# DHDev0/Stochastic-muzero

Hardware: AMD Instinct MI355X
Metric: MCTS simulations/sec (whole node), CartPole MLP 4096 envs × 50 sims (higher is better)
Workload: dtype f32 (tree values, heads) + f64 (pUCT scores, root priors) + i32 (counts)

## Files before the change

include/smz.h:

```cpp
#ifndef SMZ_H
#define SMZ_H

#include <stddef.h>
#include <stdint.h>

#ifdef __cplusplus
extern "C" {
#endif

#define SMZ_ABI_VERSION 1
#define SMZ_MAX_ACTIONS 32
#define SMZ_MAX_ACTIONS_LARGE 1024
#define SMZ_MAX_PLAYER_CYCLE 32
#define SMZ_MT_WORDS 624

typedef enum {
    SMZ_OK = 0,
    SMZ_ERR_INVALID = -1,
    SMZ_ERR_HIP = -2,
    SMZ_ERR_NOMEM = -3,
    SMZ_ERR_STATE = -4,
    SMZ_ERR_TOO_LARGE = -5
} smz_status;

// ... 65 lines not shown

int smz_expand_backup_select(smz_handle *h, const float *hidden_dev, const float *reward_dev, const float *policy_dev,
                             const float *value_dev, float *parent_hidden_dev, int32_t *last_action_dev,
                             uint8_t *branch_dev, float *mlp_input_dev, smz_stream stream);

int smz_root_stats(smz_handle *h, int32_t *visits_dev, double *priors_dev, float *root_value_dev,
                   float *child_reward_dev, smz_stream stream);

int smz_act(smz_handle *h, double temperature, const double *pow_table_host, int32_t *action_dev, double *policy_dev,
            double *child_visits_dev, float *root_value_dev, smz_stream stream);

int smz_support_decode(const float *logits_dev, int S, float *out_dev, int B, smz_stream stream);
int smz_policy_softmax(const float *logits_dev, int A, float *out_dev, int B, smz_stream stream);
int smz_dynamics_epilogue(const float *state_dyn_dev, const float *state_after_dev, const float *reward_logits_dev,
                          int ld, const uint8_t *branch_dev, int S, float *hidden_out_dev, float *reward_out_dev, int B,
                          smz_stream stream);
int smz_prediction_epilogue(const float *policy_logits_pred_dev, const float *value_logits_pred_dev,
                            const float *policy_logits_after_dev, const float *value_logits_after_dev, int ld,
                            const uint8_t *branch_dev, int A, int S, float *policy_out_dev, float *value_out_dev,
                            int B, smz_stream stream);

typedef struct {
    int32_t obs, A, S, H, L;
    int32_t OP;
    int32_t total_floats;
    int32_t off[30];
} smz_mlp_desc;
int smz_mlp_layout(smz_mlp_desc *desc);
int smz_mlp_initial(const smz_mlp_desc *desc, const float *weights_dev, const float *obs_dev, float *hidden_out_dev,
                    float *policy_out_dev, int B, smz_stream stream);
int smz_mlp_recurrent(const smz_mlp_desc *desc, const float *weights_dev, const float *mlp_input_dev,
                      const uint8_t *branch_dev, float *hidden_out_dev, float *reward_out_dev, float *policy_out_dev,
                      float *value_out_dev, int B, smz_stream stream);

enum { SMZ_LSTM_TRUNKS = 7, SMZ_LSTM_MAX_LAYERS = 4, SMZ_LSTM_REP = 2 * SMZ_LSTM_TRUNKS * SMZ_LSTM_MAX_LAYERS,
       SMZ_LSTM_OFFSETS = SMZ_LSTM_REP + 2, SMZ_LSTM_SLACK = 256 };
typedef struct {
    int32_t obs, A, S, L;
    int32_t total_floats;
    int32_t recurrent_floats;
    int32_t lds_bytes;
    int32_t off[SMZ_LSTM_OFFSETS];
} smz_lstm_desc;
int smz_lstm_layout(smz_lstm_desc *desc);
int smz_lstm_initial(const smz_lstm_desc *desc, const float *weights_dev, const float *obs_dev, float *hidden_out_dev,
                     float *policy_out_dev, int B, smz_stream stream);
int smz_lstm_recurrent(const smz_lstm_desc *desc, const float *weights_dev, const float *mlp_input_dev,
                       const uint8_t *branch_dev, float *hidden_out_dev, float *reward_out_dev, float *policy_out_dev,
                       float *value_out_dev, int B, smz_stream stream);

enum { SMZ_V_DYN = 0, SMZ_V_ADY = 1, SMZ_V_PRE = 2, SMZ_V_APR = 3 };
enum { SMZ_VT_CONV_IN = 0, SMZ_VT_BN_IN, SMZ_VT_RES_A, SMZ_VT_RES_B, SMZ_VT_RES_BN, SMZ_VT_MIX_W, SMZ_VT_MIX_B,
       SMZ_VT_TOWER , SMZ_V_TRANS_STRIDE = 13 };
enum { SMZ_VP_RES_A = 0, SMZ_VP_RES_B, SMZ_VP_RES_BN, SMZ_VP_VMIX_W, SMZ_VP_VMIX_B, SMZ_VP_VTOWER ,
       SMZ_VP_PMIX_W = 11, SMZ_VP_PMIX_B, SMZ_VP_PTOWER , SMZ_V_PRED_STRIDE = 19 };
enum { SMZ_VR_STEM = 0, SMZ_VR_NARROW_A, SMZ_VR_NARROW_B, SMZ_VR_NARROW_BN, SMZ_VR_WIDEN, SMZ_VR_WIDE_A, SMZ_VR_WIDE_B,
       SMZ_VR_WIDE_BN, SMZ_VR_LAST_A, SMZ_VR_LAST_B, SMZ_VR_LAST_BN };
enum { SMZ_V_TRANS_BASE = 0, SMZ_V_PRED_BASE = 26, SMZ_V_REP_BASE = 64, SMZ_V_OFFSETS = 80 };
typedef struct smz_vision_desc {
    int32_t A, S, H, L;
    int32_t OP;
    int32_t total_floats;
    int32_t small_floats;
    int32_t off[SMZ_V_OFFSETS];
} smz_vision_desc;
int smz_vision_layout(smz_vision_desc *desc);
// ... 141 lines not shown
```

stochastic-muzero_amd/_lib.py:

```python
import ctypes as C
import os

_HERE = os.path.dirname(os.path.abspath(__file__))
LIB_PATH = os.environ.get("SMZ_LIB_PATH") or os.path.join(_HERE, "libsmz.so")

SMZ_OK, SMZ_ERR_INVALID, SMZ_ERR_HIP, SMZ_ERR_NOMEM, SMZ_ERR_STATE, SMZ_ERR_TOO_LARGE = 0, -1, -2, -3, -4, -5
RNG_MT19937_NUMPY, RNG_PHILOX = 0, 1
MAX_ACTIONS = 32
MAX_ACTIONS_LARGE = 1024


class SmzError(RuntimeError):
    def __init__(self, code, text):
        super().__init__(f"libsmz error {code}: {text}")
        self.code = code


class Config(C.Structure):
    _fields_ = [("num_trees", C.c_int32), ("num_actions", C.c_int32), ("max_action_sample", C.c_int32),
                ("hidden_size", C.c_int32), ("num_simulations", C.c_int32), ("pb_c_base", C.c_int32),
                ("pb_c_init", C.c_double), ("discount", C.c_double), ("root_dirichlet_alpha", C.c_double),
                ("root_exploration_fraction", C.c_double), ("rng_mode", C.c_int32), ("device", C.c_int32)]


# ... 30 lines not shown


_P = C.c_void_p
SIGNATURES = {
    "smz_create": (C.c_int, [C.POINTER(Config), C.POINTER(_P)]),
    "smz_create_large_actions": (C.c_int, [C.POINTER(Config), C.POINTER(_P)]),
    "smz_destroy": (C.c_int, [_P]),
    "smz_abi_version": (C.c_int, []),
    "smz_build_features": (C.c_int, []),
    "smz_last_error": (C.c_char_p, []),
    "smz_node_capacity": (C.c_int, [_P]),
    "smz_last_kernel": (C.c_int, [_P, C.c_char_p, C.c_int]),
    "smz_set_pb_c_table": (C.c_int, [_P, _P, C.c_int]),
    "smz_seed": (C.c_int, [_P, _P, _P]),
    "smz_set_rng_state": (C.c_int, [_P, C.c_int, _P, C.c_int]),
    "smz_get_rng_state": (C.c_int, [_P, C.c_int, _P, C.POINTER(C.c_int)]),
    "smz_philox_words": (C.c_int, [C.c_uint64, C.c_uint32, C.c_int, C.c_int, _P]),
    "smz_get_philox_position": (C.c_int, [_P, C.c_int, C.POINTER(C.c_uint32), C.POINTER(C.c_int)]),
    "smz_rng_snapshot": (C.c_int, [_P, _P]),
    "smz_rng_restore": (C.c_int, [_P, _P]),
    "smz_root_init": (C.c_int, [_P, _P, _P, _P, C.c_int, _P]),
    "smz_select": (C.c_int, [_P, _P, _P, _P, _P, _P]),
    "smz_expand_backup": (C.c_int, [_P, _P, _P, _P, _P, _P]),
    "smz_expand_backup_select": (C.c_int, [_P, _P, _P, _P, _P, _P, _P, _P, _P, _P]),
    "smz_root_stats": (C.c_int, [_P, _P, _P, _P, _P, _P]),
    "smz_act": (C.c_int, [_P, C.c_double, _P, _P, _P, _P, _P, _P]),
    "smz_support_decode": (C.c_int, [_P, C.c_int, _P, C.c_int, _P]),
    "smz_policy_softmax": (C.c_int, [_P, C.c_int, _P, C.c_int, _P]),
    "smz_dynamics_epilogue": (C.c_int, [_P, _P, _P, C.c_int, _P, C.c_int, _P, _P, C.c_int, _P]),
    "smz_prediction_epilogue": (C.c_int, [_P, _P, _P, _P, C.c_int, _P, C.c_int, C.c_int, _P, _P, C.c_int, _P]),
    "smz_mlp_layout": (C.c_int, [C.POINTER(MlpDesc)]),
    "smz_mlp_initial": (C.c_int, [C.POINTER(MlpDesc), _P, _P, _P, _P, C.c_int, _P]),
    "smz_mlp_recurrent": (C.c_int, [C.POINTER(MlpDesc), _P, _P, _P, _P, _P, _P, _P, C.c_int, _P]),
    "smz_mlp_layout_wide": (C.c_int, [C.POINTER(MlpDesc)]),
    "smz_mlp_recurrent_wide": (C.c_int, [C.POINTER(MlpDesc), _P, _P, _P, _P, _P, _P, _P, C.c_int, _P]),
    "smz_mlp_layout_large": (C.c_int, [C.POINTER(MlpDesc)]),
    "smz_mlp_recurrent_large": (C.c_int, [C.POINTER(MlpDesc), _P, _P, _P, _P, _P, _P, _P, _P, C.c_int, _P]),
    "smz_mlp_initial_wide": (C.c_int, [C.POINTER(MlpDesc), _P, _P, _P, _P, C.c_int, _P]),
    "smz_mlp_initial_large": (C.c_int, [C.POINTER(MlpDesc), _P, _P, _P, _P, C.c_int, _P]),
    "smz_lstm_layout": (C.c_int, [C.POINTER(LstmDesc)]),
    "smz_lstm_initial": (C.c_int, [C.POINTER(LstmDesc), _P, _P, _P, _P, C.c_int, _P]),
    "smz_lstm_recurrent": (C.c_int, [C.POINTER(LstmDesc), _P, _P, _P, _P, _P, _P, _P, C.c_int, _P]),
    "smz_vision_layout": (C.c_int, [C.POINTER(VisionDesc)]),
    "smz_vision_initial": (C.c_int, [C.POINTER(VisionDesc), _P, _P, _P, _P, C.c_int, _P]),
    "smz_vision_initial_record": (C.c_int, [C.POINTER(VisionDesc), _P, _P, _P, _P, _P, C.c_int, _P]),
    "smz_vision_recurrent": (C.c_int, [C.POINTER(VisionDesc), _P, _P, C.c_int, _P, _P, _P, _P, _P, _P, C.c_int, _P]),
    "smz_search_mlp_act": (C.c_int, [_P, C.POINTER(MlpDesc), _P, _P, C.c_int, C.c_double, _P, _P, _P, _P, _P, _P]),
    "smz_search_mlp_act_cartpole": (C.c_int, [_P, C.POINTER(MlpDesc), _P, C.c_int, C.c_double, _P, _P, _P, _P, _P,
                                              C.POINTER(CartPoleEnv), _P]),
    "smz_search_mlp": (C.c_int, [_P, C.POINTER(MlpDesc), _P, _P, C.c_int, _P]),
    "smz_frames_resize_u8": (C.c_int, [_P, C.c_int, C.c_int, C.c_int, C.c_int, C.c_int, _P, _P, _P]),
    "smz_frames_resize_taps_u8": (C.c_int, [_P, C.c_int, C.c_int, C.c_int, C.c_int, C.c_int, _P, _P, _P]),
    "smz_host_register": (C.c_int, [_P, C.c_size_t]),
    "smz_host_unregister": (C.c_int, [_P]),
    "smz_copy_async": (C.c_int, [_P, _P, C.c_size_t, C.c_int, _P]),
    "smz_search_vision": (C.c_int, [_P, C.POINTER(VisionDesc), _P, _P, _P, C.c_int, _P]),
    "smz_search_vision_act": (C.c_int, [_P, C.POINTER(VisionDesc), _P, _P, _P, C.c_int, C.c_double, _P, _P, _P, _P, _P, _P]),
    "smz_search_lstm": (C.c_int, [_P, C.POINTER(LstmDesc), _P, _P, _P, C.c_int, _P]),
    "smz_search_lstm_act": (C.c_int, [_P, C.POINTER(LstmDesc), _P, _P, _P, C.c_int, C.c_double, _P, _P, _P, _P, _P, _P]),
    "smz_search_mlp_wide": (C.c_int, [_P, C.POINTER(MlpDesc), _P, _P, _P, C.c_int, _P]),
    "smz_search_mlp_wide_act": (C.c_int, [_P, C.POINTER(MlpDesc), _P, _P, _P, C.c_int, C.c_double, _P, _P, _P, _P, _P, _P]),
    "smz_search_mlp_large": (C.c_int, [_P, C.POINTER(MlpDesc), _P, _P, _P, C.c_int, _P]),
    "smz_search_mlp_large_act": (C.c_int, [_P, C.POINTER(MlpDesc), _P, _P, _P, C.c_int, C.c_double, _P, _P, _P, _P, _P, _P]),
    "smz_search_mlp_players": (C.c_int, [_P, C.POINTER(MlpDesc), _P, _P, C.c_int, _P]),
    "smz_search_mlp_players_act": (C.c_int, [_P, C.POINTER(MlpDesc), _P, _P, C.c_int, C.c_double, _P, _P, _P, _P, _P, _P]),
    "smz_cartpole_step": (C.c_int, [_P, _P, _P, _P, _P, C.c_int, _P]),
# ... 67 lines not shown
```

stochastic-muzero_amd/csrc/smz_mlp.hip:

```cpp
#include <hip/hip_runtime.h>
#include <math.h>
#include <stdint.h>
#include <stdlib.h>
#include <stdio.h>

#include "../../include/smz.h"
#include "smz_mlp_device.hpp"
#include "smz_mlp_wide_device.hpp"

using namespace smz_mlp;

namespace {

extern __shared__ float4 smz_mlp_lds4[];

constexpr int kFastS = 31, kFastH = 64, kFastL = 0;
template <int U, bool FASTD>
__global__ void __launch_bounds__(512) k_mlp_recurrent(smz_mlp_desc d, const float *weights, const float *x,
                                                       const uint8_t *branch, float *hidden_out, float *reward_out,
                                                       float *policy_out, float *value_out, int B, int rows_per_wave) {
    float *lds = reinterpret_cast<float *>(smz_mlp_lds4);
    stage_recurrent_weights(lds, weights, d);
    if (FASTD) { d.S = kFastS; d.H = kFastH; d.L = kFastL; d.OP = kWave; }
    const int lane = threadIdx.x & (kWave - 1), wave = threadIdx.x / kWave, waves = blockDim.x / kWave;
    float *scratch = lds + d.total_floats + wave * scratch_floats(d);
    const int row0 = (blockIdx.x * waves + wave) * rows_per_wave;
    const int S = d.S, A = d.A, K4in = up4(S + A), rs = row_scratch_floats(d);
    for (int i = 0; i < rows_per_wave; i += kRows) {
        if (row0 + i >= B) break;
        const float *xin[kRows];
        bool dyn[kRows], live[kRows];
        float *dh[kRows], *dp[kRows];
        float reward[kRows], value[kRows];
#pragma unroll
        for (int r = 0; r < kRows; r++) {
            const int row = row0 + i + r;
            live[r] = (i + r < rows_per_wave) && row < B;
            const int rr = live[r] ? row : row0 + i;
            float *xb = scratch + r * rs;
            for (int k = lane; k < K4in; k += kWave) xb[k] = (k < S + A) ? x[(size_t)rr * (S + A) + k] : 0.f;
            xin[r] = xb;
            dyn[r] = branch[rr] != 0;
            dh[r] = hidden_out + (size_t)rr * S;
            dp[r] = policy_out + (size_t)rr * A;
        }
        lds_sync();
        recurrent_rows<U, kRows>(lds, d, scratch, xin, dyn, live, dh, dp, reward, value);
#pragma unroll
        for (int r = 0; r < kRows; r++) {
            if (live[r] && lane == 0) {
                if (reward_out) reward_out[row0 + i + r] = reward[r];
                value_out[row0 + i + r] = value[r];
            }
        }
    }
}

template <int U>
__global__ void __launch_bounds__(512) k_mlp_initial(smz_mlp_desc d, const float *weights, const float *obs,
                                                     float *hidden_out, float *policy_out, int B, int rows_per_wave) {
    float *lds = reinterpret_cast<float *>(smz_mlp_lds4);
    stage_initial_weights(lds, weights, d);
    const int wave = threadIdx.x / kWave, waves = blockDim.x / kWave;
    float *scratch = lds + d.total_floats + wave * scratch_floats(d);
    const int row0 = (blockIdx.x * waves + wave) * rows_per_wave;
    for (int i = 0; i < rows_per_wave; i++) {
        const int row = row0 + i;
        if (row >= B) break;
        initial_row<U>(lds, d, lds, d, scratch, obs + (size_t)row * d.obs, hidden_out + (size_t)row * d.S, nullptr,
                       policy_out + (size_t)row * d.A);
    }
}

#ifndef SMZ_MFMA_COMPACT
#define SMZ_MFMA_COMPACT 1
#endif
constexpr bool kMfmaCompact = SMZ_MFMA_COMPACT != 0;
constexpr int kMfmaWaves = kMfmaCompact ? 16 : 12;
constexpr int kTileFloats = 32 * 32;

__device__ inline float tile_sum(const float (&a)[4][4]) {
    float s[4];
#pragma unroll
    for (int t = 0; t < 4; t++) s[t] = (a[t][0] + a[t][1]) + (a[t][2] + a[t][3]);
#pragma unroll
// ... 386 lines not shown
        const size_t lds2 = ((size_t)(kMfmaCompact ? compact_total_floats(*d) : d->total_floats - rep_floats(*d)) + (size_t)kMfmaWaves * kTileFloats) * sizeof(float) +
                            2 * kMaxChunk * sizeof(unsigned short) + 16;
        if (min_rows == 0 && lds2 > (size_t)kLdsBytes) return SMZ_ERR_TOO_LARGE;
        if (min_rows >= 0 && B >= min_rows && lds2 <= (size_t)kLdsBytes) {
            int chunk = mfma_chunk(B);
            int wgs = (B + chunk - 1) / chunk;
            if (wgs > 256) wgs = 256;
            if (d->A == 2) {
                if (allow_lds(k_mlp_recurrent_mfma<2, false>, lds2) != SMZ_OK) return SMZ_ERR_HIP;
                hipLaunchKernelGGL((k_mlp_recurrent_mfma<2, false>), dim3(wgs), dim3(kMfmaWaves * kWave), lds2, (hipStream_t)stream, *d, weights_dev,
                                   mlp_input_dev, branch_dev, hidden_out_dev, reward_out_dev, policy_out_dev, value_out_dev, B, chunk, TreeRows{});
            } else {
                if (allow_lds(k_mlp_recurrent_mfma<4, false>, lds2) != SMZ_OK) return SMZ_ERR_HIP;
                hipLaunchKernelGGL((k_mlp_recurrent_mfma<4, false>), dim3(wgs), dim3(kMfmaWaves * kWave), lds2, (hipStream_t)stream, *d, weights_dev,
                                   mlp_input_dev, branch_dev, hidden_out_dev, reward_out_dev, policy_out_dev, value_out_dev, B, chunk, TreeRows{});
            }
            return hipGetLastError() == hipSuccess ? SMZ_OK : SMZ_ERR_HIP;
        }
    }
    if (d->S == kFastS && d->H == kFastH && d->L == kFastL) {
        if (allow_lds(k_mlp_recurrent<1, true>, lds) != SMZ_OK) return SMZ_ERR_HIP;
        hipLaunchKernelGGL((k_mlp_recurrent<1, true>), dim3(blocks), dim3(kWavesPerWg * kWave), lds, (hipStream_t)stream, *d,
                           weights_dev, mlp_input_dev, branch_dev, hidden_out_dev, reward_out_dev, policy_out_dev,
                           value_out_dev, B, rpw);
    } else {
        if (allow_lds(k_mlp_recurrent<1, false>, lds) != SMZ_OK) return SMZ_ERR_HIP;
        hipLaunchKernelGGL((k_mlp_recurrent<1, false>), dim3(blocks), dim3(kWavesPerWg * kWave), lds, (hipStream_t)stream, *d,
                           weights_dev, mlp_input_dev, branch_dev, hidden_out_dev, reward_out_dev, policy_out_dev,
                           value_out_dev, B, rpw);
    }
    return hipGetLastError() == hipSuccess ? SMZ_OK : SMZ_ERR_HIP;
}

int smz_mlp_recurrent_rows(const smz_mlp_desc *d, const float *weights_dev, float *hidden_dev, int nodes_per_tree,
                           int row_stride, const int32_t *ids_dev, const int32_t *last_action_dev, const uint8_t *branch_dev,
                           float *reward_out_dev, float *policy_out_dev, float *value_out_dev, int B, smz_stream stream) {
    if (mlp_check(d, weights_dev) != SMZ_OK || !hidden_dev || !ids_dev || !last_action_dev || !branch_dev || !policy_out_dev ||
        !value_out_dev || B < 1 || nodes_per_tree < 1 || row_stride < d->S)
        return SMZ_ERR_INVALID;
    const int waves = mfma_launch_waves();
    const size_t lds2 = ((size_t)(kMfmaCompact ? compact_total_floats(*d) : d->total_floats - rep_floats(*d)) + (size_t)waves * kTileFloats) * sizeof(float) +
                        2 * kMaxChunk * sizeof(unsigned short) + 16;
    if (!(d->S == kFastS && d->H == kFastH && d->L == kFastL && (d->A == 2 || d->A == 4)) || lds2 > (size_t)kLdsBytes)
        return SMZ_ERR_TOO_LARGE;
    int chunk = mfma_chunk(B);
    int wgs = (B + chunk - 1) / chunk;
    if (wgs > 256) wgs = 256;
    const TreeRows tr = {hidden_dev, ids_dev, last_action_dev, nodes_per_tree, row_stride};
    if (d->A == 2) {
        if (allow_lds(k_mlp_recurrent_mfma<2, true>, lds2) != SMZ_OK) return SMZ_ERR_HIP;
        hipLaunchKernelGGL((k_mlp_recurrent_mfma<2, true>), dim3(wgs), dim3(waves * kWave), lds2, (hipStream_t)stream, *d, weights_dev,
                           nullptr, branch_dev, nullptr, reward_out_dev, policy_out_dev, value_out_dev, B, chunk, tr);
    } else {
        if (allow_lds(k_mlp_recurrent_mfma<4, true>, lds2) != SMZ_OK) return SMZ_ERR_HIP;
        hipLaunchKernelGGL((k_mlp_recurrent_mfma<4, true>), dim3(wgs), dim3(waves * kWave), lds2, (hipStream_t)stream, *d, weights_dev,
                           nullptr, branch_dev, nullptr, reward_out_dev, policy_out_dev, value_out_dev, B, chunk, tr);
    }
    return hipGetLastError() == hipSuccess ? SMZ_OK : SMZ_ERR_HIP;
}

int smz_mlp_layout_wide(smz_mlp_desc *d) {
    if (!d || d->obs < 1 || d->A < 1 || d->S < 1 || d->H < 1 || d->L < 0) return SMZ_ERR_INVALID;
    if (d->H > kWideOP || 2 * d->S > kWideOP || d->A + d->S > kWideOP) return SMZ_ERR_TOO_LARGE;
    d->OP = kWideOP;
    const int mid = d->L > 0 ? d->H : 0;
    const int K[M_COUNT] = {d->S + d->A, d->S + d->A, mid, mid, d->H, d->H, d->S, d->S, mid, mid, d->H, d->H, d->obs, mid, d->H};
// ... 32 lines not shown
```

stochastic-muzero_amd/csrc/smz_mlp_device.hpp:

```cpp
#pragma once
#include <hip/hip_runtime.h>
#include <math.h>
#include <stdint.h>

#include "../../include/smz.h"

namespace smz_mlp {

constexpr int kWave = 64;
enum { M_DYN_IN, M_ADY_IN, M_DYN_MID, M_ADY_MID, M_DYN_OUT, M_ADY_OUT, M_PRE_IN, M_APR_IN, M_PRE_MID, M_APR_MID,
       M_PRE_OUT, M_APR_OUT, M_REP_IN, M_REP_MID, M_REP_OUT, M_COUNT };

__host__ __device__ inline int up4(int x) { return (x + 3) & ~3; }

typedef float v2f __attribute__((ext_vector_type(2)));
__device__ inline v2f pk_fma(float wx, float wy, float ax, float ay, v2f c) {
    v2f w = {wx, wy}, a = {ax, ay};
    return __builtin_elementwise_fma(w, a, c);
}
template <int U, int R, bool SAME = false>
__device__ inline void dense(const float *const (&W)[R], const float *const (&bias)[R], const float *const (&act)[R], int K4,
                             const int (&OP)[R], int lane, float (&acc)[R][U]) {
    const float4 *a4[R], *w4[R];
    v2f acc2[R][U];
// ... 30 lines not shown
                }
            }
        }
    }
    for (; q < n; q++) {
#pragma unroll
        for (int r = 0; r < R; r++) {
            const float4 av = a4[r][q];
#pragma unroll
            for (int u = 0; u < U; u++) {
                const float4 wv = w4[SAME ? 0 : r][(size_t)q * OP[SAME ? 0 : r] + kWave * u];
                v2f t = acc2[r][u];
                t = pk_fma(wv.x, wv.y, av.x, av.y, t);
                t = pk_fma(wv.z, wv.w, av.z, av.w, t);
                acc2[r][u] = t;
            }
        }
    }
#pragma unroll
    for (int r = 0; r < R; r++)
#pragma unroll
        for (int u = 0; u < U; u++) acc[r][u] = acc2[r][u].x + acc2[r][u].y;
}

template <int U, int R, bool SAME = false>
__device__ inline void dense(const float *const (&W)[R], const float *const (&bias)[R], const float *const (&act)[R], int K4,
                             int OP, int lane, float (&acc)[R][U]) {
    int op[R];
#pragma unroll
    for (int r = 0; r < R; r++) op[r] = OP;
    dense<U, R, SAME>(W, bias, act, K4, op, lane, acc);
}

__device__ inline float dense_halves(const float *W, const float *bias, const float *act0, const float *act1, int K4, int OP, int lane) {
    const int o = lane & 31;
    const float4 *a4 = reinterpret_cast<const float4 *>(lane < 32 ? act0 : act1);
    const float4 *w4 = reinterpret_cast<const float4 *>(W) + o;
    v2f acc2 = {bias[o], 0.f};
    const int n = K4 >> 2;
    int q = 0;
    for (; q + 4 <= n; q += 4) {
        float4 a[4], w[4];
#pragma unroll
        for (int j = 0; j < 4; j++) { a[j] = a4[q + j]; w[j] = w4[(size_t)(q + j) * OP]; }
#pragma unroll
        for (int j = 0; j < 4; j++) {
            acc2 = pk_fma(w[j].x, w[j].y, a[j].x, a[j].y, acc2);
            acc2 = pk_fma(w[j].z, w[j].w, a[j].z, a[j].w, acc2);
        }
    }
    for (; q < n; q++) {
        const float4 av = a4[q], wv = w4[(size_t)q * OP];
        acc2 = pk_fma(wv.x, wv.y, av.x, av.y, acc2);
        acc2 = pk_fma(wv.z, wv.w, av.z, av.w, acc2);
    }
    return acc2.x + acc2.y;
}

__device__ inline float smz_exp(float x) { return __expf(x); }
__device__ inline float elu(float x) { return x > 0.f ? x : smz_exp(x) - 1.0f; }
#ifndef SMZ_DPP_VOLATILE
#define SMZ_DPP_VOLATILE volatile
#endif
#ifndef SMZ_PAIR_TAILS
#define SMZ_PAIR_TAILS 1
#endif
#ifndef SMZ_ONE_DECODE
#define SMZ_ONE_DECODE 1
#endif
#ifndef SMZ_DENSE_HALVES
#define SMZ_DENSE_HALVES 1
#endif
#define SMZ_DPP_REDUCE(NAME, INSN)                                                               \
    __device__ inline float NAME(float v) {                                                      \
        asm SMZ_DPP_VOLATILE("s_nop 1\n\t"                                                               \
                     INSN " %0, %0, %0 row_shr:1 row_mask:0xf bank_mask:0xf\n\ts_nop 1\n\t"      \
                     INSN " %0, %0, %0 row_shr:2 row_mask:0xf bank_mask:0xf\n\ts_nop 1\n\t"      \
                     INSN " %0, %0, %0 row_shr:4 row_mask:0xf bank_mask:0xf\n\ts_nop 1\n\t"      \
                     INSN " %0, %0, %0 row_shr:8 row_mask:0xf bank_mask:0xf\n\ts_nop 1\n\t"      \
                     INSN " %0, %0, %0 row_bcast:15 row_mask:0xa bank_mask:0xf\n\ts_nop 1\n\t"   \
                     INSN " %0, %0, %0 row_bcast:31 row_mask:0xc bank_mask:0xf\n\ts_nop 1"        \
                     : "+v"(v));                                                                 \
        return __int_as_float(__builtin_amdgcn_readlane(__float_as_int(v), 63));                 \
    }
SMZ_DPP_REDUCE(wave_max, "v_max_f32_dpp")
SMZ_DPP_REDUCE(wave_min, "v_min_f32_dpp")
SMZ_DPP_REDUCE(wave_sum, "v_add_f32_dpp")
#undef SMZ_DPP_REDUCE
__device__ inline float op_max(float a, float b) { return fmaxf(a, b); }
__device__ inline float op_min(float a, float b) { return fminf(a, b); }
__device__ inline void wave_sum2(float &a, float &b) {
    asm SMZ_DPP_VOLATILE("s_nop 1\n\t"
                 "v_add_f32_dpp %0, %0, %0 row_shr:1 row_mask:0xf bank_mask:0xf\n\tv_add_f32_dpp %1, %1, %1 row_shr:1 row_mask:0xf bank_mask:0xf\n\ts_nop 0\n\t"
                 "v_add_f32_dpp %0, %0, %0 row_shr:2 row_mask:0xf bank_mask:0xf\n\tv_add_f32_dpp %1, %1, %1 row_shr:2 row_mask:0xf bank_mask:0xf\n\ts_nop 0\n\t"
                 "v_add_f32_dpp %0, %0, %0 row_shr:4 row_mask:0xf bank_mask:0xf\n\tv_add_f32_dpp %1, %1, %1 row_shr:4 row_mask:0xf bank_mask:0xf\n\ts_nop 0\n\t"
                 "v_add_f32_dpp %0, %0, %0 row_shr:8 row_mask:0xf bank_mask:0xf\n\tv_add_f32_dpp %1, %1, %1 row_shr:8 row_mask:0xf bank_mask:0xf\n\ts_nop 0\n\t"
                 "v_add_f32_dpp %0, %0, %0 row_bcast:15 row_mask:0xa bank_mask:0xf\n\tv_add_f32_dpp %1, %1, %1 row_bcast:15 row_mask:0xa bank_mask:0xf\n\ts_nop 0\n\t"
                 "v_add_f32_dpp %0, %0, %0 row_bcast:31 row_mask:0xc bank_mask:0xf\n\tv_add_f32_dpp %1, %1, %1 row_bcast:31 row_mask:0xc bank_mask:0xf\n\ts_nop 1"
                 : "+v"(a), "+v"(b));
    a = __int_as_float(__builtin_amdgcn_readlane(__float_as_int(a), 63));
    b = __int_as_float(__builtin_amdgcn_readlane(__float_as_int(b), 63));
}
__device__ inline void wave_minmax(float &mn, float &mx) {
    asm SMZ_DPP_VOLATILE("s_nop 1\n\t"
// ... 175 lines not shown
    const float s0 = __int_as_float(__builtin_amdgcn_readlane(__float_as_int(v), 31));
    const float s1 = __int_as_float(__builtin_amdgcn_readlane(__float_as_int(v), 63));
    return hi ? s1 : s0;
}
#define SMZ_HSTEP1(I0, CTRL) I0 " %0, %0, %0 " CTRL "\n\t"
#define SMZ_HSTEP2(I0, I1, CTRL) I0 " %0, %0, %0 " CTRL "\n\t" I1 " %1, %1, %1 " CTRL "\n\t"
#define SMZ_HSTEP3(I0, I1, I2, CTRL) I0 " %0, %0, %0 " CTRL "\n\t" I1 " %1, %1, %1 " CTRL "\n\t" I2 " %2, %2, %2 " CTRL "\n\t"
#define SMZ_HSTEP5(I, CTRL) I " %0, %0, %0 " CTRL "\n\t" I " %1, %1, %1 " CTRL "\n\t" I " %2, %2, %2 " CTRL "\n\t" I " %3, %3, %3 " CTRL "\n\t" I " %4, %4, %4 " CTRL "\n\t"
#define SMZ_HALF_CHAIN(STEP, ...)                                                          \
    "s_nop 1\n\t" STEP(__VA_ARGS__, "row_shr:1 row_mask:0xf bank_mask:0xf") "s_nop 0\n\t"  \
    STEP(__VA_ARGS__, "row_shr:2 row_mask:0xf bank_mask:0xf") "s_nop 0\n\t"                \
    STEP(__VA_ARGS__, "row_shr:4 row_mask:0xf bank_mask:0xf") "s_nop 0\n\t"                \
    STEP(__VA_ARGS__, "row_shr:8 row_mask:0xf bank_mask:0xf") "s_nop 0\n\t"                \
    STEP(__VA_ARGS__, "row_bcast:15 row_mask:0xa bank_mask:0xf") "s_nop 1"
__device__ inline void half_max2(float &a, float &b) {
    asm SMZ_DPP_VOLATILE(SMZ_HALF_CHAIN(SMZ_HSTEP2, "v_max_f32_dpp", "v_max_f32_dpp") : "+v"(a), "+v"(b));
}
__device__ inline void half_minmax(float &mn, float &mx) {
    asm SMZ_DPP_VOLATILE(SMZ_HALF_CHAIN(SMZ_HSTEP2, "v_min_f32_dpp", "v_max_f32_dpp") : "+v"(mn), "+v"(mx));
}
__device__ inline void half_max_min_max(float &a, float &b, float &c) {
    asm SMZ_DPP_VOLATILE(SMZ_HALF_CHAIN(SMZ_HSTEP3, "v_max_f32_dpp", "v_min_f32_dpp", "v_max_f32_dpp") : "+v"(a), "+v"(b), "+v"(c));
}
__device__ inline void half_sum2(float &a, float &b) {
    asm SMZ_DPP_VOLATILE(SMZ_HALF_CHAIN(SMZ_HSTEP2, "v_add_f32_dpp", "v_add_f32_dpp") : "+v"(a), "+v"(b));
}
__device__ inline void half_sum3(float &a, float &b, float &c) {
    asm SMZ_DPP_VOLATILE(SMZ_HALF_CHAIN(SMZ_HSTEP3, "v_add_f32_dpp", "v_add_f32_dpp", "v_add_f32_dpp") : "+v"(a), "+v"(b), "+v"(c));
}
__device__ inline void half_sum5(float &a, float &b, float &c, float &d, float &e) {
    asm SMZ_DPP_VOLATILE(SMZ_HALF_CHAIN(SMZ_HSTEP5, "v_add_f32_dpp") : "+v"(a), "+v"(b), "+v"(c), "+v"(d), "+v"(e));
}

template <bool WITH_REWARD = false>
__device__ inline void softmax_decode_pair(float a0, float a1, int A, int S, int lane, float *dst0, float *dst1, float &val0,
                                           float &val1, float rnum = 0.f, float rden = 0.f, float *rew0 = nullptr, float *rew1 = nullptr) {
    float P = a0, Q = a1;
    swap32(P, Q);
    const bool hi = lane >= 32;
    const int j = lane & 31, oq = 32 + j, half = S / 2;
    const bool ppol = j < A, pval = !ppol && j < A + S, qval = oq >= A && oq < A + S;
    float mp = ppol ? P : -__builtin_inff();
    float mv = op_max(pval ? P : -__builtin_inff(), qval ? Q : -__builtin_inff());
    half_max2(mp, mv);
    mp = half_bcast(mp, hi); mv = half_bcast(mv, hi);
    const float eP = (ppol || pval) ? smz_exp(P - (ppol ? mp : mv)) : 0.f;
    const float eQ = qval ? smz_exp(Q - mv) : 0.f;
    float dp = ppol ? eP : 0.f, dvP = pval ? eP : 0.f, nvP = pval ? (float)(j - A - half) * eP : 0.f;
    float dv, nv;
    if (A + S == 33) {
        half_sum3(dp, dvP, nvP);
        int q = __builtin_amdgcn_update_dpp(0, __float_as_int(eQ), 0x140, 0xf, 0xf, false);
        q = __builtin_amdgcn_update_dpp(q, q, 0x142, 0xa, 0xf, false);
        const float e32 = __int_as_float(q);
        dv = dvP + e32;
        nv = nvP + (float)(32 - A - half) * e32;
    } else {
        float dvQ = eQ, nvQ = qval ? (float)(oq - A - half) * eQ : 0.f;
        half_sum5(dp, dvP, nvP, dvQ, nvQ);
        dv = dvP + dvQ; nv = nvP + nvQ;
    }
    if constexpr (WITH_REWARD) {
        const float sn = __int_as_float(__builtin_amdgcn_update_dpp(0, __float_as_int(rnum), 0x101, 0xf, 0xf, false));
        const float sd = __int_as_float(__builtin_amdgcn_update_dpp(0, __float_as_int(rden), 0x101, 0xf, 0xf, false));
        const bool rl = (lane & 31) == 30;
        nv = rl ? sn : nv;
        dv = rl ? sd : dv;
    }
    const float v = support_to_scalar(nv, dv);
    val0 = __int_as_float(__builtin_amdgcn_readlane(__float_as_int(v), 31));
    val1 = __int_as_float(__builtin_amdgcn_readlane(__float_as_int(v), 63));
    if constexpr (WITH_REWARD) {
        *rew0 = __int_as_float(__builtin_amdgcn_readlane(__float_as_int(v), 30));
        *rew1 = __int_as_float(__builtin_amdgcn_readlane(__float_as_int(v), 62));
    }
    const float dpb = half_bcast(dp, hi);
    float *dst = hi ? dst1 : dst0;
    if (ppol && dst) dst[j] = __fdividef(eP, dpb);
}

template <bool DEFER = false>
__device__ inline void dynamics_tail_pair(float a0, float a1, bool d0, bool d1, int S, int lane, float *act0, float *act1,
                                          float *dst0, float *dst1, float &rew0, float &rew1, float *rnum = nullptr, float *rden = nullptr) {
    float P = a0, Q = a1;
    swap32(P, Q);
    const bool hi = lane >= 32, dyn = hi ? d1 : d0;
    const int j = lane & 31, oq = 32 + j, half = S / 2;
    const bool plog = dyn && j < S;
    const bool pst = dyn ? (j >= S && j < 2 * S) : j < S, qst = dyn && oq < 2 * S;
    float mr = plog ? P : -__builtin_inff();
    float mn = op_min(pst ? P : __builtin_inff(), qst ? Q : __builtin_inff());
    float mx = op_max(pst ? P : -__builtin_inff(), qst ? Q : -__builtin_inff());
    half_max_min_max(mr, mn, mx);
    mr = half_bcast(mr, hi); mn = half_bcast(mn, hi); mx = half_bcast(mx, hi);
    const float e = plog ? smz_exp(P - mr) : 0.f;
    float den = e, num = plog ? (float)(j - half) * e : 0.f;
    half_sum2(den, num);
    if constexpr (DEFER) {
        *rnum = num; *rden = den;
        rew0 = rew1 = 0.f;
    } else {
        const float r = support_to_scalar(num, den);
        rew0 = d0 ? __int_as_float(__builtin_amdgcn_readlane(__float_as_int(r), 31)) : 0.f;
        rew1 = d1 ? __int_as_float(__builtin_amdgcn_readlane(__float_as_int(r), 63)) : 0.f;
    }
    float sc = mx - mn;
    if (sc < 1e-5f) sc += 1e-5f;
    float *act = hi ? act1 : act0, *dst = hi ? dst1 : dst0;
    const int ip = dyn ? j - S : j;
    if (pst) { const float h = __fdividef(P - mn, sc); act[ip] = h; if (dst) dst[ip] = h; }
    if (qst) { const float h = __fdividef(Q - mn, sc); act[oq - S] = h; if (dst) dst[oq - S] = h; }
}

template <bool PACKED = false>
__device__ inline void scale_pair(float a0, float a1, int S, int lane, float *act0, float *act1, float *dst0, float *dst1) {
    float P = a0, Q = a1;
    if (!PACKED) swap32(P, Q);
    const bool hi = lane >= 32;
// ... 64 lines not shown
        lds_sync();
    }
}

__device__ inline void stage_weights(float *lds, const float *weights, const int *ranges, int n_ranges) {
    constexpr int UB = 8;
    for (int r = 0; r < n_ranges; r++) {
        const int off = ranges[2 * r], cnt = ranges[2 * r + 1];
        for (int i0 = threadIdx.x * 4; i0 < cnt; i0 += blockDim.x * 4 * UB) {
            float4 v[UB];
#pragma unroll
            for (int u = 0; u < UB; u++) {
                const int i = i0 + u * blockDim.x * 4;
                v[u] = *reinterpret_cast<const float4 *>(weights + off + (i < cnt ? i : i0));
            }
#pragma unroll
            for (int u = 0; u < UB; u++) {
                const int i = i0 + u * blockDim.x * 4;
                if (i < cnt) *reinterpret_cast<float4 *>(lds + off + i) = v[u];
            }
        }
    }
    __syncthreads();
}

constexpr int kRows = 1;

__host__ __device__ inline int row_scratch_floats(const smz_mlp_desc &d) {
    const int kin = up4(d.S + d.A) > up4(d.obs) ? up4(d.S + d.A) : up4(d.obs);
    return kin + up4(d.H) + up4(d.S);
}
__host__ __device__ inline int scratch_floats(const smz_mlp_desc &d) { return kRows * row_scratch_floats(d); }

template <int U, int R, bool SAME = false, bool CP = false>
__device__ inline void recurrent_rows(const float *lds, const smz_mlp_desc &d, float *scratch, const float *const (&xin)[R],
                                      const bool (&dyn)[R], const bool (&live)[R], float *const (&dst_hidden)[R],
                                      float *const (&dst_policy)[R], float (&reward)[R], float (&value)[R]) {
    const int S = d.S, A = d.A, K4in = up4(S + A), K4h = up4(d.H), K4s = up4(S);
    const int lane = threadIdx.x & (kWave - 1);
    const int rs = row_scratch_floats(d), kin = rs - K4h - K4s;
    float *tA[R], *hbuf[R];
    MatOff m1[R], m1m[R], m3[R], m3m[R];
#pragma unroll
    for (int r = 0; r < R; r++) {
        tA[r] = scratch + r * rs + kin;
        hbuf[r] = tA[r] + K4h;
        m1[r] = pick<CP>(d, dyn[r], M_DYN_IN, M_ADY_IN);   m1m[r] = pick<CP>(d, dyn[r], M_DYN_MID, M_ADY_MID);
        m3[r] = pick<CP>(d, dyn[r], M_PRE_IN, M_APR_IN);   m3m[r] = pick<CP>(d, dyn[r], M_PRE_MID, M_APR_MID);
        for (int k = lane; k < K4s; k += kWave) hbuf[r][k] = 0.f;
    }
    trunk<U, R, SAME>(lds, d, m1, m1m, xin, K4in, tA, lane);
    float acc[R][U];
    constexpr bool PAIRED = SMZ_PAIR_TAILS && U == 1 && R == 2;
    const bool halves = PAIRED && SAME && SMZ_DENSE_HALVES && S <= 32 && !dyn[0] && !dyn[1];
    if (halves) {
        if constexpr (PAIRED && SAME) {
            const MatOff m = pick<CP>(d, false, M_DYN_OUT, M_ADY_OUT);
            acc[0][0] = dense_halves(lds + m.w, lds + m.b, tA[0], tA[1], K4h, m.op, lane);
            acc[1][0] = 0.f;
        }
    } else {
        const float *W[R], *Bv[R], *Ac[R];
        int op[R];
#pragma unroll
        for (int r = 0; r < R; r++) {
            const MatOff m = pick<CP>(d, dyn[r], M_DYN_OUT, M_ADY_OUT);
            W[r] = lds + m.w; Bv[r] = lds + m.b; Ac[r] = tA[r]; op[r] = m.op;
        }
        dense<U, R, SAME>(W, Bv, Ac, K4h, op, lane, acc);
    }
    float pair_rnum = 0.f, pair_rden = 0.f;
    bool pair_reward = false;
    if constexpr (PAIRED) {
        if (S <= 32) {
            reward[0] = reward[1] = 0.f;
            if (halves) scale_pair<true>(acc[0][0], 0.f, S, lane, hbuf[0], hbuf[1], live[0] ? dst_hidden[0] : nullptr,
                                         live[1] ? dst_hidden[1] : nullptr);
            else if (!dyn[0] && !dyn[1]) scale_pair(acc[0][0], acc[1][0], S, lane, hbuf[0], hbuf[1], live[0] ? dst_hidden[0] : nullptr,
                                               live[1] ? dst_hidden[1] : nullptr);
            else if (SMZ_ONE_DECODE) {
                dynamics_tail_pair<true>(acc[0][0], acc[1][0], dyn[0], dyn[1], S, lane, hbuf[0], hbuf[1], live[0] ? dst_hidden[0] : nullptr,
                                         live[1] ? dst_hidden[1] : nullptr, reward[0], reward[1], &pair_rnum, &pair_rden);
                pair_reward = true;
            } else dynamics_tail_pair(acc[0][0], acc[1][0], dyn[0], dyn[1], S, lane, hbuf[0], hbuf[1], live[0] ? dst_hidden[0] : nullptr,
                                      live[1] ? dst_hidden[1] : nullptr, reward[0], reward[1]);
        } else {
#pragma unroll
            for (int r = 0; r < R; r++) {
                reward[r] = 0.f;
                if (dyn[r]) reward[r] = decode_scale_lanes<U>(acc[r], S, lane, hbuf[r], live[r] ? dst_hidden[r] : nullptr);
                else scale_lanes<U>(acc[r], 0, S, lane, hbuf[r], live[r] ? dst_hidden[r] : nullptr);
            }
        }
    } else {
#pragma unroll
    for (int r = 0; r < R; r++) {
        reward[r] = 0.f;
        if (dyn[r]) {
            reward[r] = decode_scale_lanes<U>(acc[r], S, lane, hbuf[r], live[r] ? dst_hidden[r] : nullptr);
        } else {
            scale_lanes<U>(acc[r], 0, S, lane, hbuf[r], live[r] ? dst_hidden[r] : nullptr);
        }
    }
    }
    lds_sync();
    {
        const float *Hc[R];
#pragma unroll
        for (int r = 0; r < R; r++) Hc[r] = hbuf[r];
        trunk<U, R, SAME>(lds, d, m3, m3m, Hc, K4s, tA, lane);
        const float *W[R], *Bv[R], *Ac[R];
        int op[R];
#pragma unroll
// ... 138 lines not shown
```

stochastic-muzero_amd/csrc/smz_search_mlp.hpp:

```cpp
#pragma once
#include "smz_common.hpp"
#include "smz_handle.hpp"

namespace {

extern __shared__ float4 smz_search_lds4[];

#ifndef SMZ_BPS_HBM
#define SMZ_BPS_HBM 1
#endif
#ifndef SMZ_SELECT_BLOCKS
#define SMZ_SELECT_BLOCKS 1
#endif
#ifndef SMZ_EARLY_ROWS
#define SMZ_EARLY_ROWS 1
#endif
#ifndef SMZ_PAIR_A4
#define SMZ_PAIR_A4 1
#endif
#ifndef SMZ_SELECT_TWO_PASSES
#define SMZ_SELECT_TWO_PASSES 1
#endif
#ifndef SMZ_LEAF_FIRST
#define SMZ_LEAF_FIRST 1
// ... 418 lines not shown
        __builtin_amdgcn_s_setprio(SMZ_PRIO_HEADS);
        if (!(BPS && SMZ_EARLY_ROWS && bps_all)) __builtin_amdgcn_fence(__ATOMIC_SEQ_CST, "workgroup");
        if (split && !(dbg & 8) && !staged_early) stage_issue<SU, PHC>(P, tree, valid, packed, pre);
        if (BPS && SMZ_EARLY_ROWS && bps_all) {
#pragma unroll
            for (int t = 0; t < kFastTpw; t++) {
                if (tree0 + t >= P.B) break;
                const int act = __builtin_amdgcn_readlane(L.action, t);
                if (lane < K4in) xall[t * K4in + lane] = (lane < S) ? early_row[t] : ((lane < S + A && (lane - S) == act) ? 1.f : 0.f);
            }
        } else
        for (int t = 0; t < tpw; t++) {
            const int row = tree0 + t;
            if (row >= P.B) break;
            const int parent = __builtin_amdgcn_readlane(L.parent_id, t), act = __builtin_amdgcn_readlane(L.action, t);
            const float *src = P.hidden + ((size_t)row * P.N + parent) * P.hs;
            for (int k = lane; k < K4in; k += kWave)
                xall[t * K4in + k] = (k < S) ? src[k] : ((k < S + A && (k - S) == act) ? 1.f : 0.f);
        }
        smz_mlp::lds_sync();
        SMZ_PROBE_B(3)
        bool paired = false;
        if (tpw == 2 && !(dbg & 1)) {
            const int b0 = __builtin_amdgcn_readlane(L.branch, 0), b1 = __builtin_amdgcn_readlane(L.branch, 1);
            if (tree0 + 1 < P.B) {
                const float *xin[2] = {xall, xall + K4in};
                const bool dyn[2] = {b0 != 0, b1 != 0};
                float *dh[2], *dp[2] = {outs, outs + slot};
                float reward[2], value[2];
#pragma unroll
                for (int r = 0; r < 2; r++)
                    dh[r] = P.hidden + ((size_t)(tree0 + r) * P.N + __builtin_amdgcn_readlane(L.leaf_id, r)) * P.hs;
                const bool live[2] = {MSK ? (vmask & 1) != 0 : true, MSK ? (vmask & 2) != 0 : true};
                if (b0 == b1) smz_mlp::recurrent_rows<U, 2, true, TLDS>(lds, dl, scratch, xin, dyn, live, dh, dp, reward, value);
                else smz_mlp::recurrent_rows<U, 2, false, TLDS>(lds, dl, scratch, xin, dyn, live, dh, dp, reward, value);
                SMZ_PROBE_B(4)
                if (lane == 0) {
                    outs[A] = value[0]; outs[A + 1] = reward[0];
                    outs[slot + A] = value[1]; outs[slot + A + 1] = reward[1];
                }
                paired = true;
            }
        }
        for (int t = 0; t < tpw && !paired; t += smz_mlp::kRows) {
            if (tree0 + t >= P.B) break;
            constexpr int R = smz_mlp::kRows;
            const float *xin[R];
            bool dyn[R], live[R];
            float *dh[R], *dp[R];
            float reward[R], value[R];
#pragma unroll
            for (int r = 0; r < R; r++) {
                live[r] = (t + r < tpw) && (tree0 + t + r < P.B);
                const int tt = live[r] ? t + r : t;
                live[r] = live[r] && (!MSK || __shfl((int)valid, tt) != 0);
                const int row = tree0 + tt;
                const int leaf = __builtin_amdgcn_readlane(L.leaf_id, tt);
                dyn[r] = __builtin_amdgcn_readlane(L.branch, tt) != 0;
                xin[r] = xall + tt * K4in;
                dh[r] = P.hidden + ((size_t)row * P.N + leaf) * P.hs;
                dp[r] = outs + tt * slot;
            }
            if (!(dbg & 1)) smz_mlp::recurrent_rows<U, R, false, TLDS>(lds, dl, scratch, xin, dyn, live, dh, dp, reward, value);
#pragma unroll
            for (int r = 0; r < R; r++)
                if (live[r] && lane == 0) { outs[(t + r) * slot + A] = value[r]; outs[(t + r) * slot + A + 1] = reward[r]; }
        }
// ... 140 lines not shown
```

Baseline: 538.8 million.

## Run paired recurrent rows on wave halves with multi-output dense

Adds a half-wave path for paired recurrent inference: each 32-lane half of the wave computes one tree's row, and a new dense_rows_halves computes two output columns per lane. The pair path is used when the two rows take different branches (dynamics vs afterstate) and the network is small (S<=32, H<=64, OP=64). It is meant to avoid running both branch weight sets over the whole wave in the mixed case. The softmax/dynamics tails get a PACKED mode that skips the swap32, since outputs already sit in their halves. A standalone pairs kernel and API are also added. The cost is more LDS syncs per layer and twice the per-lane weight loads.

```diff
diff --git a/include/smz.h b/include/smz.h
--- a/include/smz.h
+++ b/include/smz.h
@@ -121,6 +121,9 @@
 int smz_mlp_recurrent(const smz_mlp_desc *desc, const float *weights_dev, const float *mlp_input_dev,
                       const uint8_t *branch_dev, float *hidden_out_dev, float *reward_out_dev, float *policy_out_dev,
                       float *value_out_dev, int B, smz_stream stream);
+int smz_mlp_recurrent_pairs(const smz_mlp_desc *desc, const float *weights_dev, const float *mlp_input_dev,
+                            const uint8_t *branch_dev, float *hidden_out_dev, float *reward_out_dev, float *policy_out_dev,
+                            float *value_out_dev, int B, int compact_image, smz_stream stream);
 
 enum { SMZ_LSTM_TRUNKS = 7, SMZ_LSTM_MAX_LAYERS = 4, SMZ_LSTM_REP = 2 * SMZ_LSTM_TRUNKS * SMZ_LSTM_MAX_LAYERS,
        SMZ_LSTM_OFFSETS = SMZ_LSTM_REP + 2, SMZ_LSTM_SLACK = 256 };
diff --git a/stochastic-muzero_amd/_lib.py b/stochastic-muzero_amd/_lib.py
--- a/stochastic-muzero_amd/_lib.py
+++ b/stochastic-muzero_amd/_lib.py
@@ -86,6 +86,7 @@
     "smz_mlp_layout": (C.c_int, [C.POINTER(MlpDesc)]),
     "smz_mlp_initial": (C.c_int, [C.POINTER(MlpDesc), _P, _P, _P, _P, C.c_int, _P]),
     "smz_mlp_recurrent": (C.c_int, [C.POINTER(MlpDesc), _P, _P, _P, _P, _P, _P, _P, C.c_int, _P]),
+    "smz_mlp_recurrent_pairs": (C.c_int, [C.POINTER(MlpDesc), _P, _P, _P, _P, _P, _P, _P, C.c_int, C.c_int, _P]),
     "smz_mlp_layout_wide": (C.c_int, [C.POINTER(MlpDesc)]),
     "smz_mlp_recurrent_wide": (C.c_int, [C.POINTER(MlpDesc), _P, _P, _P, _P, _P, _P, _P, C.c_int, _P]),
     "smz_mlp_layout_large": (C.c_int, [C.POINTER(MlpDesc)]),
diff --git a/stochastic-muzero_amd/csrc/smz_mlp.hip b/stochastic-muzero_amd/csrc/smz_mlp.hip
--- a/stochastic-muzero_amd/csrc/smz_mlp.hip
+++ b/stochastic-muzero_amd/csrc/smz_mlp.hip
@@ -51,6 +51,49 @@
             if (live[r] && lane == 0) {
                 if (reward_out) reward_out[row0 + i + r] = reward[r];
                 value_out[row0 + i + r] = value[r];
+            }
+        }
+    }
+}
+
+template <bool CP>
+__global__ void __launch_bounds__(512) k_mlp_recurrent_pairs(smz_mlp_desc d, const float *weights, const float *x,
+                                                             const uint8_t *branch, float *hidden_out, float *reward_out,
+                                                             float *policy_out, float *value_out, int B, int pairs_per_wave) {
+    float *lds = reinterpret_cast<float *>(smz_mlp_lds4);
+    const smz_mlp_desc dl = CP ? lds_desc_compact(d) : d;
+    if (CP) stage_weights_compact(lds, weights, d);
+    else stage_recurrent_weights(lds, weights, d);
+    const int lane = threadIdx.x & (kWave - 1), wave = threadIdx.x / kWave, waves = blockDim.x / kWave;
+    const int S = d.S, A = d.A, K4in = up4(S + A), rs = row_scratch_floats(d);
+    float *scratch = lds + ((dl.total_floats + 3) & ~3) + wave * 2 * rs;
+    const int pair0 = (blockIdx.x * waves + wave) * pairs_per_wave;
+    for (int i = 0; i < pairs_per_wave; i++) {
+        const int row0 = 2 * (pair0 + i);
+        if (row0 >= B) break;
+        const float *xin[2];
+        bool dyn[2], live[2];
+        float *dh[2], *dp[2];
+        float reward[2], value[2];
+#pragma unroll
+        for (int r = 0; r < 2; r++) {
+            live[r] = row0 + r < B;
+            const int rr = live[r] ? row0 + r : row0;
+            float *xb = scratch + r * rs;
+            for (int k = lane; k < K4in; k += kWave) xb[k] = (k < S + A) ? x[(size_t)rr * (S + A) + k] : 0.f;
+            xin[r] = xb;
+            dyn[r] = __builtin_amdgcn_readfirstlane((int)branch[rr]) != 0;
+            dh[r] = hidden_out + (size_t)rr * S;
+            dp[r] = policy_out + (size_t)rr * A;
+        }
+        lds_sync();
+        if (SMZ_PAIR_HALVES < 2 && dyn[0] == dyn[1]) recurrent_rows<1, 2, true, CP>(lds, dl, scratch, xin, dyn, live, dh, dp, reward, value);
+        else recurrent_rows<1, 2, false, CP>(lds, dl, scratch, xin, dyn, live, dh, dp, reward, value);
+#pragma unroll
+        for (int r = 0; r < 2; r++) {
+            if (live[r] && lane == 0) {
+                if (reward_out) reward_out[row0 + r] = reward[r];
+                value_out[row0 + r] = value[r];
             }
         }
     }
@@ -503,6 +546,31 @@
     return hipGetLastError() == hipSuccess ? SMZ_OK : SMZ_ERR_HIP;
 }
 
+int smz_mlp_recurrent_pairs(const smz_mlp_desc *d, const float *weights_dev, const float *mlp_input_dev,
+                            const uint8_t *branch_dev, float *hidden_out_dev, float *reward_out_dev, float *policy_out_dev,
+                            float *value_out_dev, int B, int compact_image, smz_stream stream) {
+    if (mlp_check(d, weights_dev) != SMZ_OK || !mlp_input_dev || !branch_dev || !hidden_out_dev || !policy_out_dev ||
+        !value_out_dev || B < 1)
+        return SMZ_ERR_INVALID;
+    const int pairs = (B + 1) / 2;
+    int ppw = (pairs + 256 * kWavesPerWg - 1) / (256 * kWavesPerWg);
+    if (ppw < 1) ppw = 1;
+    const int blocks = (pairs + ppw * kWavesPerWg - 1) / (ppw * kWavesPerWg);
+    const int image = compact_image ? compact_total_floats(*d) : d->total_floats;
+    const size_t lds = ((size_t)((image + 3) & ~3) + (size_t)kWavesPerWg * 2 * row_scratch_floats(*d)) * sizeof(float);
+    if (lds > (size_t)kLdsBytes) return SMZ_ERR_TOO_LARGE;
+    if (compact_image) {
+        if (allow_lds(k_mlp_recurrent_pairs<true>, lds) != SMZ_OK) return SMZ_ERR_HIP;
+        hipLaunchKernelGGL((k_mlp_recurrent_pairs<true>), dim3(blocks), dim3(kWavesPerWg * kWave), lds, (hipStream_t)stream, *d,
+                           weights_dev, mlp_input_dev, branch_dev, hidden_out_dev, reward_out_dev, policy_out_dev, value_out_dev, B, ppw);
+    } else {
+        if (allow_lds(k_mlp_recurrent_pairs<false>, lds) != SMZ_OK) return SMZ_ERR_HIP;
+        hipLaunchKernelGGL((k_mlp_recurrent_pairs<false>), dim3(blocks), dim3(kWavesPerWg * kWave), lds, (hipStream_t)stream, *d,
+                           weights_dev, mlp_input_dev, branch_dev, hidden_out_dev, reward_out_dev, policy_out_dev, value_out_dev, B, ppw);
+    }
+    return hipGetLastError() == hipSuccess ? SMZ_OK : SMZ_ERR_HIP;
+}
+
 int smz_mlp_recurrent_rows(const smz_mlp_desc *d, const float *weights_dev, float *hidden_dev, int nodes_per_tree,
                            int row_stride, const int32_t *ids_dev, const int32_t *last_action_dev, const uint8_t *branch_dev,
                            float *reward_out_dev, float *policy_out_dev, float *value_out_dev, int B, smz_stream stream) {
diff --git a/stochastic-muzero_amd/csrc/smz_mlp_device.hpp b/stochastic-muzero_amd/csrc/smz_mlp_device.hpp
--- a/stochastic-muzero_amd/csrc/smz_mlp_device.hpp
+++ b/stochastic-muzero_amd/csrc/smz_mlp_device.hpp
@@ -86,29 +86,55 @@
     dense<U, R, SAME>(W, bias, act, K4, op, lane, acc);
 }
 
-__device__ inline float dense_halves(const float *W, const float *bias, const float *act0, const float *act1, int K4, int OP, int lane) {
+template <int NO>
+__device__ inline void dense_rows_halves(const float *W, const float *bias, const float *act, int K4, int OP, int lane, float (&acc)[NO]) {
     const int o = lane & 31;
-    const float4 *a4 = reinterpret_cast<const float4 *>(lane < 32 ? act0 : act1);
-    const float4 *w4 = reinterpret_cast<const float4 *>(W) + o;
-    v2f acc2 = {bias[o], 0.f};
+    const float4 *a4 = reinterpret_cast<const float4 *>(act);
+    const float4 *wp = reinterpret_cast<const float4 *>(W) + o;
+    v2f acc2[NO];
+#pragma unroll
+    for (int u = 0; u < NO; u++) { acc2[u].x = bias[o + 32 * u]; acc2[u].y = 0.f; }
     const int n = K4 >> 2;
     int q = 0;
     for (; q + 4 <= n; q += 4) {
-        float4 a[4], w[4];
-#pragma unroll
-        for (int j = 0; j < 4; j++) { a[j] = a4[q + j]; w[j] = w4[(size_t)(q + j) * OP]; }
+        float4 a[4], w[NO][4];
 #pragma unroll
         for (int j = 0; j < 4; j++) {
-            acc2 = pk_fma(w[j].x, w[j].y, a[j].x, a[j].y, acc2);
-            acc2 = pk_fma(w[j].z, w[j].w, a[j].z, a[j].w, acc2);
+            a[j] = a4[q + j];
+#pragma unroll
+            for (int u = 0; u < NO; u++) w[u][j] = wp[32 * u];
+            wp += OP;
+        }
+#pragma unroll
+        for (int j = 0; j < 4; j++) {
+#pragma unroll
+            for (int u = 0; u < NO; u++) {
+                v2f t = acc2[u];
+                t = pk_fma(w[u][j].x, w[u][j].y, a[j].x, a[j].y, t);
+                t = pk_fma(w[u][j].z, w[u][j].w, a[j].z, a[j].w, t);
+                acc2[u] = t;
+            }
         }
     }
     for (; q < n; q++) {
-        const float4 av = a4[q], wv = w4[(size_t)q * OP];
-        acc2 = pk_fma(wv.x, wv.y, av.x, av.y, acc2);
-        acc2 = pk_fma(wv.z, wv.w, av.z, av.w, acc2);
-    }
-    return acc2.x + acc2.y;
+        const float4 av = a4[q];
+#pragma unroll
+        for (int u = 0; u < NO; u++) {
+            const float4 wv = wp[32 * u];
+            v2f t = acc2[u];
+            t = pk_fma(wv.x, wv.y, av.x, av.y, t);
+            t = pk_fma(wv.z, wv.w, av.z, av.w, t);
+            acc2[u] = t;
+        }
+        wp += OP;
+    }
+#pragma unroll
+    for (int u = 0; u < NO; u++) acc[u] = acc2[u].x + acc2[u].y;
+}
+__device__ inline float dense_halves(const float *W, const float *bias, const float *act0, const float *act1, int K4, int OP, int lane) {
+    float acc[1];
+    dense_rows_halves<1>(W, bias, lane < 32 ? act0 : act1, K4, OP, lane, acc);
+    return acc[0];
 }
 
 __device__ inline float smz_exp(float x) { return __expf(x); }
@@ -124,6 +150,9 @@
 #endif
 #ifndef SMZ_DENSE_HALVES
 #define SMZ_DENSE_HALVES 1
+#endif
+#ifndef SMZ_PAIR_HALVES
+#define SMZ_PAIR_HALVES 1
 #endif
 #define SMZ_DPP_REDUCE(NAME, INSN)                                                               \
     __device__ inline float NAME(float v) {                                                      \
@@ -365,11 +394,11 @@
     asm SMZ_DPP_VOLATILE(SMZ_HALF_CHAIN(SMZ_HSTEP5, "v_add_f32_dpp") : "+v"(a), "+v"(b), "+v"(c), "+v"(d), "+v"(e));
 }
 
-template <bool WITH_REWARD = false>
+template <bool WITH_REWARD = false, bool PACKED = false>
 __device__ inline void softmax_decode_pair(float a0, float a1, int A, int S, int lane, float *dst0, float *dst1, float &val0,
                                            float &val1, float rnum = 0.f, float rden = 0.f, float *rew0 = nullptr, float *rew1 = nullptr) {
     float P = a0, Q = a1;
-    swap32(P, Q);
+    if (!PACKED) swap32(P, Q);
     const bool hi = lane >= 32;
     const int j = lane & 31, oq = 32 + j, half = S / 2;
     const bool ppol = j < A, pval = !ppol && j < A + S, qval = oq >= A && oq < A + S;
@@ -412,11 +441,11 @@
     if (ppol && dst) dst[j] = __fdividef(eP, dpb);
 }
 
-template <bool DEFER = false>
+template <bool DEFER = false, bool PACKED = false>
 __device__ inline void dynamics_tail_pair(float a0, float a1, bool d0, bool d1, int S, int lane, float *act0, float *act1,
                                           float *dst0, float *dst1, float &rew0, float &rew1, float *rnum = nullptr, float *rden = nullptr) {
     float P = a0, Q = a1;
-    swap32(P, Q);
+    if (!PACKED) swap32(P, Q);
     const bool hi = lane >= 32, dyn = hi ? d1 : d0;
     const int j = lane & 31, oq = 32 + j, half = S / 2;
     const bool plog = dyn && j < S;
@@ -547,10 +576,80 @@
 }
 __host__ __device__ inline int scratch_floats(const smz_mlp_desc &d) { return kRows * row_scratch_floats(d); }
 
+template <bool CP, int MA, int MB>
+__device__ inline void halves_elu_layer(const float *lds, const smz_mlp_desc &d, bool dynh, const float *act, int K4, float *tA,
+                                        int lane, bool in_place) {
+    const MatOff m = pick<CP>(d, dynh, MA, MB);
+    float acc[2];
+    dense_rows_halves<2>(lds + m.w, lds + m.b, act, K4, m.op, lane, acc);
+    if (in_place) lds_sync();
+#pragma unroll
+    for (int u = 0; u < 2; u++) { const int o = (lane & 31) + 32 * u; if (o < up4(d.H)) tA[o] = (o < d.H) ? elu(acc[u]) : 0.f; }
+    lds_sync();
+}
+
+template <bool CP>
+__device__ inline void recurrent_pair_halves(const float *lds, const smz_mlp_desc &d, float *scratch, const float *const (&xin)[2],
+                                             const bool (&dyn)[2], const bool (&live)[2], float *const (&dst_hidden)[2],
+                                             float *const (&dst_policy)[2], float (&reward)[2], float (&value)[2]) {
+    const int S = d.S, A = d.A, K4in = up4(S + A), K4h = up4(d.H), K4s = up4(S);
+    const int lane = threadIdx.x & (kWave - 1);
+    const bool hi = lane >= 32, dynh = hi ? dyn[1] : dyn[0];
+    const int rs = row_scratch_floats(d), kin = rs - K4h - K4s;
+    float *tA = scratch + (hi ? rs : 0) + kin;
+    float *hbuf0 = scratch + kin + K4h, *hbuf1 = hbuf0 + rs, *hbuf = hi ? hbuf1 : hbuf0;
+    for (int k = lane & 31; k < K4s; k += 32) hbuf[k] = 0.f;
+    halves_elu_layer<CP, M_DYN_IN, M_ADY_IN>(lds, d, dynh, hi ? xin[1] : xin[0], K4in, tA, lane, false);
+    for (int l = 0; l < d.L; l++) halves_elu_layer<CP, M_DYN_MID, M_ADY_MID>(lds, d, dynh, tA, K4h, tA, lane, true);
+    float *const dh0 = live[0] ? dst_hidden[0] : nullptr, *const dh1 = live[1] ? dst_hidden[1] : nullptr;
+    float acc[2];
+    float pair_rnum = 0.f, pair_rden = 0.f;
+    bool pair_reward = false;
+    reward[0] = reward[1] = 0.f;
+    const MatOff mo = pick<CP>(d, dynh, M_DYN_OUT, M_ADY_OUT);
+    if (SMZ_PAIR_HALVES > 1 && !dyn[0] && !dyn[1]) {
+        acc[0] = dense_halves(lds + mo.w, lds + mo.b, tA, tA, K4h, mo.op, lane);
+        scale_pair<true>(acc[0], 0.f, S, lane, hbuf0, hbuf1, dh0, dh1);
+    } else {
+        dense_rows_halves<2>(lds + mo.w, lds + mo.b, tA, K4h, mo.op, lane, acc);
+        if (SMZ_ONE_DECODE && A <= 32) {
+            dynamics_tail_pair<true, true>(acc[0], acc[1], dyn[0], dyn[1], S, lane, hbuf0, hbuf1, dh0, dh1, reward[0], reward[1],
+                                           &pair_rnum, &pair_rden);
+            pair_reward = true;
+        } else dynamics_tail_pair<false, true>(acc[0], acc[1], dyn[0], dyn[1], S, lane, hbuf0, hbuf1, dh0, dh1, reward[0], reward[1]);
+    }
+    lds_sync();
+    halves_elu_layer<CP, M_PRE_IN, M_APR_IN>(lds, d, dynh, hbuf, K4s, tA, lane, false);
+    for (int l = 0; l < d.L; l++) halves_elu_layer<CP, M_PRE_MID, M_APR_MID>(lds, d, dynh, tA, K4h, tA, lane, true);
+    const MatOff mp = pick<CP>(d, dynh, M_PRE_OUT, M_APR_OUT);
+    dense_rows_halves<2>(lds + mp.w, lds + mp.b, tA, K4h, mp.op, lane, acc);
+    float *const dp0 = live[0] ? dst_policy[0] : nullptr, *const dp1 = live[1] ? dst_policy[1] : nullptr;
+    if (A <= 32 && pair_reward) {
+        float r0, r1;
+        softmax_decode_pair<true, true>(acc[0], acc[1], A, S, lane, dp0, dp1, value[0], value[1], pair_rnum, pair_rden, &r0, &r1);
+        reward[0] = dyn[0] ? r0 : 0.f;
+        reward[1] = dyn[1] ? r1 : 0.f;
+    } else if (A <= 32) {
+        softmax_decode_pair<false, true>(acc[0], acc[1], A, S, lane, dp0, dp1, value[0], value[1]);
+    } else {
+        swap32(acc[0], acc[1]);
+        const float a0[1] = {acc[0]}, a1[1] = {acc[1]};
+        value[0] = softmax_decode_lanes<1>(a0, A, S, lane, dp0);
+        value[1] = softmax_decode_lanes<1>(a1, A, S, lane, dp1);
+    }
+    lds_sync();
+}
+
 template <int U, int R, bool SAME = false, bool CP = false>
 __device__ inline void recurrent_rows(const float *lds, const smz_mlp_desc &d, float *scratch, const float *const (&xin)[R],
                                       const bool (&dyn)[R], const bool (&live)[R], float *const (&dst_hidden)[R],
                                       float *const (&dst_policy)[R], float (&reward)[R], float (&value)[R]) {
+    if constexpr (SMZ_PAIR_TAILS && U == 1 && R == 2 && (SMZ_PAIR_HALVES > 1 || (SMZ_PAIR_HALVES == 1 && !SAME))) {
+        if (d.S <= 32 && d.H <= 64 && d.A + d.S <= 64 && d.OP == kWave) {
+            recurrent_pair_halves<CP>(lds, d, scratch, xin, dyn, live, dst_hidden, dst_policy, reward, value);
+            return;
+        }
+    }
     const int S = d.S, A = d.A, K4in = up4(S + A), K4h = up4(d.H), K4s = up4(S);
     const int lane = threadIdx.x & (kWave - 1);
     const int rs = row_scratch_floats(d), kin = rs - K4h - K4s;
@@ -593,7 +692,7 @@
                                          live[1] ? dst_hidden[1] : nullptr);
             else if (!dyn[0] && !dyn[1]) scale_pair(acc[0][0], acc[1][0], S, lane, hbuf[0], hbuf[1], live[0] ? dst_hidden[0] : nullptr,
                                                live[1] ? dst_hidden[1] : nullptr);
-            else if (SMZ_ONE_DECODE) {
+            else if (SMZ_ONE_DECODE && A <= 32) {
                 dynamics_tail_pair<true>(acc[0][0], acc[1][0], dyn[0], dyn[1], S, lane, hbuf[0], hbuf[1], live[0] ? dst_hidden[0] : nullptr,
                                          live[1] ? dst_hidden[1] : nullptr, reward[0], reward[1], &pair_rnum, &pair_rden);
                 pair_reward = true;
diff --git a/stochastic-muzero_amd/csrc/smz_search_mlp.hpp b/stochastic-muzero_amd/csrc/smz_search_mlp.hpp
--- a/stochastic-muzero_amd/csrc/smz_search_mlp.hpp
+++ b/stochastic-muzero_amd/csrc/smz_search_mlp.hpp
@@ -474,7 +474,7 @@
                 for (int r = 0; r < 2; r++)
                     dh[r] = P.hidden + ((size_t)(tree0 + r) * P.N + __builtin_amdgcn_readlane(L.leaf_id, r)) * P.hs;
                 const bool live[2] = {MSK ? (vmask & 1) != 0 : true, MSK ? (vmask & 2) != 0 : true};
-                if (b0 == b1) smz_mlp::recurrent_rows<U, 2, true, TLDS>(lds, dl, scratch, xin, dyn, live, dh, dp, reward, value);
+                if (SMZ_PAIR_HALVES < 2 && b0 == b1) smz_mlp::recurrent_rows<U, 2, true, TLDS>(lds, dl, scratch, xin, dyn, live, dh, dp, reward, value);
                 else smz_mlp::recurrent_rows<U, 2, false, TLDS>(lds, dl, scratch, xin, dyn, live, dh, dp, reward, value);
                 SMZ_PROBE_B(4)
                 if (lane == 0) {
```

After: 552.0 million, median of 6. +2.5%, better.
